# AberHu/TF-NAS

Measured on AMD Instinct MI355X. Metric: supernet search images/sec (w-step + alpha-step), higher is better.
Workload: dtype fp32

## Files before the change

include/tfnas_hip.h:

```cpp
#ifndef TFNAS_HIP_H
#define TFNAS_HIP_H

#include <stddef.h>
#include <stdint.h>

#ifdef __cplusplus
extern "C" {
#endif

#define TFNAS_ABI_VERSION 4
#define TFNAS_MAX_GROUPS 8
#define TFNAS_MAX_SINK 4
#define TFNAS_MAX_CELLS 32

#define TFNAS_MODE_CELL 0
#define TFNAS_MODE_STEM 1
#define TFNAS_MODE_HEAD 2

#define TFNAS_ACT_RELU 0
#define TFNAS_ACT_SWISH 1

#define TFNAS_EINVAL (-1)
#define TFNAS_ENULL (-2)
#define TFNAS_ERANGE (-3)
// ... 1 lines not shown
typedef struct TfnasGroup {
    int32_t mc;
    int32_t k;
    int32_t se;
    int32_t mcp;
    int32_t off;
    int32_t se_off;
    int32_t pad0, pad1;
    const float *w_expand, *w_dw, *w_proj, *w_se_r, *b_se_r, *w_se_e, *b_se_e;
    float *g_expand, *g_dw, *g_proj, *g_se_r, *gb_se_r, *g_se_e, *gb_se_e;
} TfnasGroup;

typedef struct TfnasCellDesc {
    int32_t N, H, W;
    int32_t ic, oc;
    int32_t stride;
    int32_t act;
    int32_t has_res;
    int32_t G;
    int32_t need_wgrad;
    int32_t Ho, Wo;
    int32_t M;
    int32_t SE;
    float eps;
    int32_t mode;
    int32_t Hi, Wi;
    int32_t stor;
    int32_t gemm_mode;
    int32_t flags;
    TfnasGroup g[TFNAS_MAX_GROUPS];
    int (*sync_fn)(void *user, double *table, uint64_t ndoubles, void *stream);
    void *sync_user;
    int32_t sync_world;
    int32_t route;
    int32_t fwd_route;
    int32_t pad_route;
    void *wgrad_stream[3];
} TfnasCellDesc;
#define TFNAS_GEMM_EXPLICIT 0x1000
#define TFNAS_CELL_LAZY_JOIN 1
#define TFNAS_CELL_ACCUM_WGRAD 0x20
#define TFNAS_ROUTE_FX_OFF 0x1
#define TFNAS_ROUTE_FOLD_OFF 0x2
#define TFNAS_ROUTE_DWWG_OFF 0x4
#define TFNAS_ROUTE_DWWG2_OFF 0x8
#define TFNAS_ROUTE_XG_OFF 0x10
#define TFNAS_ROUTE_XG_ALL 0x20
#define TFNAS_ROUTE_DW_SHIFT 6
#define TFNAS_ROUTE_DW_MASK 0xc0
#define TFNAS_ROUTE_SE_SHIFT 8
#define TFNAS_ROUTE_SE_MASK 0x300
#define TFNAS_ROUTE_WGRAD_INLINE 0x400
#define TFNAS_ROUTE_GRAM2 0x800
#define TFNAS_ROUTE_ALL 0xfff
#define TFNAS_ROUTE_TAKEN_VALID 0x1
#define TFNAS_ROUTE_TAKEN_FX 0x2

typedef struct TfnasCellWs {
    uint64_t E;
    uint64_t D;
    uint64_t Pr;
    uint64_t fsmall;
    uint64_t off_pooled, off_gate, off_hpre;
    uint64_t stats;
    uint64_t off_stats1, off_stats2, off_stats3;
    uint64_t out;
    uint64_t dZ;
    uint64_t dEh;
    uint64_t bsmall;
    uint64_t off_dgate, off_dpooled, off_dgl, off_dhpre, off_cb1;
    uint64_t red;
    uint64_t off_red3, off_red2, off_red1, off_resdot;
    uint64_t part;
    uint64_t dx;
    uint64_t dxp;
} TfnasCellWs;

int tfnas_abi_version(void);

typedef int (*tfnas_stats_sync_fn)(void *user, double *table, uint64_t ndoubles, void *stream);
int tfnas_set_stats_sync(tfnas_stats_sync_fn fn, void *user, int world);

int tfnas_shutdown(void);

uint64_t tfnas_sizeof(int which);

int tfnas_cell_plan(TfnasCellDesc *d);

int tfnas_cell_ws(const TfnasCellDesc *d, TfnasCellWs *ws);

int tfnas_efree_supported(const TfnasCellDesc *d);
int tfnas_cell_route(const TfnasCellDesc *d);
int tfnas_fx_supported(const TfnasCellDesc *d);

int tfnas_mixedop_fwd(const TfnasCellDesc *d, const float *x, const float *wmix,
                      float *E, float *D, float *Pr, float *fsmall, double *stats, float *part,
                      float *out, void *stream);

int tfnas_mixedop_bwd(const TfnasCellDesc *d, const float *x, const float *wmix,
                      const float *E, const float *D, const float *Pr, const float *fsmall,
                      const double *stats, const float *dout,
                      float *dZ, float *dEh, float *bsmall, double *red, float *part,
                      float *dx, float *dxp, float *dwmix, void *stream);

typedef struct TfnasBnAffine {
    const float *weight[3], *bias[3];
    float *g_weight[3], *g_bias[3];
// ... 136 lines not shown
```

tf-nas_amd/csrc/gemm_core.h:

```cpp
#pragma once
#include "tfnas_dev.h"

template <int NT>
struct GT {
    static constexpr int BM = 128, BK = 16, BN = 16 * NT;
    static constexpr int LDA = BM + 16;
    static constexpr int LDB = (BN % 32 == 16) ? BN : BN + 16;
    static constexpr int A_FLOATS = BK * LDA, B_FLOATS = BK * LDB;
    static constexpr int X3_FLOATS = 1584 * NT;
    static constexpr int LDS_FLOATS = 2 * (A_FLOATS + B_FLOATS) > X3_FLOATS ? 2 * (A_FLOATS + B_FLOATS) : X3_FLOATS;
    static constexpr int B_ITEMS = BN * 4;
    static constexpr int B_ITERS = (B_ITEMS + 255) / 256;
};

template <int NT>
__device__ __forceinline__ void acc_zero(f32x4 (&acc)[2][NT]) {
#pragma unroll
    for (int i = 0; i < 2; ++i)
#pragma unroll
        for (int j = 0; j < NT; ++j) acc[i][j] = zero4();
}

struct XfId {
    __device__ __forceinline__ f32x4 operator()(f32x4 v, int, int, int, int) const { return v; }
// ... 42 lines not shown
        _Pragma("unroll") for (int i = 0; i < T::B_ITERS; ++i) {                            \
            TFNAS_B_IDX(i);                                                                 \
            if (idx < T::B_ITEMS) {                                                         \
                const f32x4 v = xb(rb[i], (c), i, b0_, b1_);                                   \
                if (BKC) {                                                                  \
                    (Bs)[(b1_ + 0) * T::LDB + b0_] = v.x;                                   \
                    (Bs)[(b1_ + 1) * T::LDB + b0_] = v.y;                                   \
                    (Bs)[(b1_ + 2) * T::LDB + b0_] = v.z;                                   \
                    (Bs)[(b1_ + 3) * T::LDB + b0_] = v.w;                                   \
                } else {                                                                    \
                    st4(&(Bs)[b0_ * T::LDB + b1_], v);                                      \
                }                                                                           \
            }                                                                               \
        }                                                                                   \
    }

    float* As0 = lds;
    float* As1 = lds + T::A_FLOATS;
    float* Bs0 = lds + 2 * T::A_FLOATS;
    float* Bs1 = Bs0 + T::B_FLOATS;
#define TFNAS_MFMAS(As, Bs)                                                                 \
    _Pragma("unroll") for (int ks = 0; ks < 4; ++ks) {                                      \
        const int k = ks * 4 + lk;                                                          \
        const float a0 = (As)[k * T::LDA + wrow + lr];                                      \
        const float a1 = (As)[k * T::LDA + wrow + 16 + lr];                                 \
        _Pragma("unroll") for (int j = 0; j < NT; ++j) {                                    \
            const float b = (Bs)[k * T::LDB + 16 * j + lr];                                 \
            acc[0][j] = __builtin_amdgcn_mfma_f32_16x16x4f32(a0, b, acc[0][j], 0, 0, 0);    \
            acc[1][j] = __builtin_amdgcn_mfma_f32_16x16x4f32(a1, b, acc[1][j], 0, 0, 0);    \
        }                                                                                   \
    }

    if (nchunks > 0) {
        TFNAS_GLOAD(0);
        TFNAS_SSTORE(0, As0, Bs0);
    }
    __syncthreads();
    for (int c = 0; c < nchunks; ++c) {
        const bool more = (c + 1 < nchunks);
        if (more) TFNAS_GLOAD(c + 1);
        if (c & 1) { TFNAS_MFMAS(As1, Bs1); } else { TFNAS_MFMAS(As0, Bs0); }
        if (more) {
            if (c & 1) { TFNAS_SSTORE(c + 1, As0, Bs0); } else { TFNAS_SSTORE(c + 1, As1, Bs1); }
        }
        __syncthreads();
    }
#undef TFNAS_MFMAS
#undef TFNAS_GLOAD
#undef TFNAS_SSTORE
#undef TFNAS_A_IDX
#undef TFNAS_B_IDX
}

struct PreNone {
    __device__ __forceinline__ void operator()(int) const {}
};
template <int NT, bool BKC, class PRE, class LA, class XA, class LB, class XB>
__device__ __forceinline__ void gemm_mainloop_adirect(PRE& pre, LA& la, XA& xa, LB& lb, XB& xb, int nchunks,
                                                      f32x4 (&acc)[2][NT], float* lds) {
    using T = GT<NT>;
    using RA = decltype(la(0, 0, 0));
    using RB = decltype(lb(0, 0, 0));
    const int tid = threadIdx.x, lane = tid & 63;
    const int lr = lane & 15, lk = lane >> 4;
    RA ra[2];
    RB rb[T::B_ITERS];
    f32x4 cur[2];

#define TFNAS_B_IDX(i)                                                      \
    const int idx = tid + 256 * (i), b0_ = BKC ? (idx >> 2) : idx / (T::BN / 4), \
              b1_ = BKC ? (idx & 3) * 4 : (idx % (T::BN / 4)) * 4
#define TFNAS_GLOAD(c)                                                                      \
    {                                                                                       \
        pre(c);                                                                             \
        _Pragma("unroll") for (int i = 0; i < 2; ++i) ra[i] = la((c), i, 4 * lk);           \
        _Pragma("unroll") for (int i = 0; i < T::B_ITERS; ++i) {                            \
            TFNAS_B_IDX(i);                                                                 \
            if (idx < T::B_ITEMS) rb[i] = lb((c), b0_, b1_);                                \
        }                                                                                   \
    }
#define TFNAS_SSTORE(c, Bs)                                                                 \
    {                                                                                       \
        _Pragma("unroll") for (int i = 0; i < 2; ++i) cur[i] = xa(ra[i], (c), i, 4 * lk);   \
        _Pragma("unroll") for (int i = 0; i < T::B_ITERS; ++i) {                            \
            TFNAS_B_IDX(i);                                                                 \
            if (idx < T::B_ITEMS) {                                                         \
                const f32x4 v = xb(rb[i], (c), b0_, b1_);                                   \
                if (BKC) {                          \
                    const int r0_ = b1_ >> 2;                                               \
                    (Bs)[(r0_ + 0) * T::LDB + b0_] = v.x;                                   \
                    (Bs)[(r0_ + 4) * T::LDB + b0_] = v.y;                                   \
                    (Bs)[(r0_ + 8) * T::LDB + b0_] = v.z;                                   \
                    (Bs)[(r0_ + 12) * T::LDB + b0_] = v.w;                                  \
                } else {                                                                    \
                    st4(&(Bs)[((b0_ & 3) * 4 + (b0_ >> 2)) * T::LDB + b1_], v);             \
                }                                                                           \
            }                                                                               \
        }                                                                                   \
    }

    float* Bs0 = lds;
    float* Bs1 = lds + T::B_FLOATS;
    if (nchunks > 0) {
        TFNAS_GLOAD(0);
        TFNAS_SSTORE(0, Bs0);
    }
// ... 124 lines not shown
```

tf-nas_amd/csrc/gemm_kernels.hip:

```cpp
#include <stdlib.h>
#include <string.h>
#include "gemm_core.h"
#include "gemm_x3.h"
#include "kernels.h"
#include "prof.h"

__device__ __forceinline__ f32x4 stem_patch4(const float* __restrict__ img, const TfnasCellDesc& d, int p, int t0) {
    const int HW = d.H * d.W, n = p / HW, r = p - n * HW, ho = r / d.W, wo = r - ho * d.W;
    f32x4 v = zero4();
#pragma unroll
    for (int j = 0; j < 4; ++j) {
        const int t = t0 + j;
        if (t < 27) {
            const int ci = t / 9, rem = t - 9 * ci, ky = rem / 3, kx = rem - 3 * ky;
            const int hi = 2 * ho + ky - 1, wi = 2 * wo + kx - 1;
            if (hi >= 0 && hi < d.Hi && wi >= 0 && wi < d.Wi) v[j] = img[((size_t)(n * 3 + ci) * d.Hi + hi) * d.Wi + wi];
        }
    }
    return v;
}

constexpr int kLbBig = 3, kLbSmall = 4;
constexpr int kLbX3Big = 2, kLbX3Small = 3;
constexpr int gemm_lb(int nt, int mm) { return mm == 0 ? (nt >= 5 ? kLbBig : kLbSmall) : (nt >= 5 ? kLbX3Big : kLbX3Small); }
// ... 385 lines not shown
            const int pw0 = rt * 128 + w * 32;
            const int imgA = min(pw0, Po - 1) / HW, bnd = (imgA + 1) * HW;
            float sum[2][FOLD_Q][NC];
#pragma unroll
            for (int a = 0; a < 2; ++a)
#pragma unroll
                for (int q = 0; q < FOLD_Q; ++q)
#pragma unroll
                    for (int c = 0; c < NC; ++c) sum[a][q][c] = 0.f;
            const float* Dcol = D + off + n0;
            emit_tile_rows<NT>(acc, lds,
                               [&](int lrow, int lc, f32x4 v) {
                                   const int p = rt * 128 + lrow;
                                   if (p < Po && n0 + lc < mcp) st4_nt(dZ + ((size_t)p * M + off + n0 + lc), v);
                               },
                               [&](int i, const float* st) {
                                   if (d.act == TFNAS_ACT_RELU)
                                       fold_slab<NT, TFNAS_ACT_RELU>(st, LDC, Dcol, M, pw0 + 16 * i, Po, bnd, c2f, cokf, has_se, sum);
                                   else
                                       fold_slab<NT, TFNAS_ACT_SWISH>(st, LDC, Dcol, M, pw0 + 16 * i, Po, bnd, c2f, cokf, has_se, sum);
                               });
            static_assert(4 * 2 * FOLD_Q * T::BN + 4 <= T::LDS_FLOATS, "fold staging does not fit the GEMM LDS buffer");
            float* comb = lds;
            int* meta = reinterpret_cast<int*>(lds + 4 * 2 * FOLD_Q * T::BN);
#pragma unroll
            for (int a = 0; a < 2; ++a)
#pragma unroll
                for (int q = 0; q < FOLD_Q; ++q)
#pragma unroll
                    for (int c = 0; c < NC; ++c)
                        if (lane + 64 * c < T::BN) comb[((w * 2 + a) * FOLD_Q + q) * T::BN + lane + 64 * c] = sum[a][q][c];
            if (lane == 0) meta[w] = imgA;
            __syncthreads();
            const int img0 = min(rt * 128, Po - 1) / HW, imgL = min(rt * 128 + 127, Po - 1) / HW;
            const int nq = has_se ? FOLD_Q : 2;
            for (int o = tid; o < FOLD_SLOTS * FOLD_Q * T::BN; o += 256) {
                const int sl = o / (FOLD_Q * T::BN), q = (o / T::BN) % FOLD_Q, col = o % T::BN;
                if (img0 + sl > imgL || q >= nq || n0 + col >= mcp) continue;
                float t = 0.f;
#pragma unroll
                for (int ww = 0; ww < 4; ++ww)
#pragma unroll
                    for (int a = 0; a < 2; ++a)
                        if (meta[ww] + a - img0 == sl) t += comb[((ww * 2 + a) * FOLD_Q + q) * T::BN + col];
                rec[(((size_t)rt * FOLD_SLOTS + sl) * FOLD_Q + q) * M + off + n0 + col] = t;
            }
            __syncthreads();
        }
    }
}

constexpr int wgrad_lb(int nt) { return nt >= 5 ? 2 : (nt >= 3 ? 3 : 4); }

template <int NT, int ACT>
__global__ __launch_bounds__(256, wgrad_lb(NT)) void k_project_wgrad(TfnasCellDesc d, const float* __restrict__ dout,
                                                       const float* __restrict__ Pr, const float* __restrict__ D,
                                                       const float* __restrict__ gate,
                                                       const double* __restrict__ stats2,
                                                       const double* __restrict__ stats3,
                                                       const double* __restrict__ red3,
                                                       const float* __restrict__ wmix, int rows_per_split,
                                                       int ntiles_o, float* __restrict__ part, size_t out_size) {
    using T = GT<NT>;
    extern __shared__ __attribute__((aligned(16))) float lds[];
    const int g = blockIdx.z / ntiles_o, n0 = (blockIdx.z % ntiles_o) * T::BN;
    const int mc = d.g[g].mc, mcp = d.g[g].mcp, off = d.g[g].off;
    const bool has_se = d.g[g].se > 0;
    const float* gbase = has_se ? gate : D;
    const size_t se01 = has_se ? 1 : 0;
    size_t poff = 0;
    for (int gg = 0; gg < g; ++gg) poff += (size_t)d.g[gg].mc * d.oc;
    float* __restrict__ gw = part + (size_t)blockIdx.x * out_size + poff;
    const int m0 = blockIdx.y * 128;
    if (m0 >= mcp) return;
    const int HW = d.Ho * d.Wo, Po = d.N * HW, oc = d.oc, M = d.M;
    const int ocp = (oc + 15) & ~15;
    const int r0 = blockIdx.x * rows_per_split, r1 = min(Po, r0 + rows_per_split);
    const int nchunks = (r1 - r0 + 15) >> 4;
    const int tid = threadIdx.x, lane = tid & 63, lr = lane & 15, lq = lane >> 4, wrow = (tid >> 6) * 32;

    const Bn3Tab tab = bn3_tab_fill(lds + T::LDS_FLOATS, ocp, d, g, stats3, red3, wmix);
    const int mch = m0 + (tid & 31) * 4;
    const bool chok = mch < mcp;
    const size_t acol = (size_t)off + min(mch, mcp - 4);
    float2 c2[4];
#pragma unroll
    for (int j = 0; j < 4; ++j)
        c2[j] = (mch + j < mc) ? bn_consts(stats2 + 2 * (size_t)(off + mch + j), 1.0 / (double)Po, d.eps)
                               : make_float2(0.f, 0.f);
    __syncthreads();
    constexpr int BQ = T::BN / 4;
    int bcol[T::B_ITERS];
    bool bok[T::B_ITERS];
    f32x4 k_mean[T::B_ITERS], k_a3[T::B_ITERS], k_ab[T::B_ITERS], k_s[T::B_ITERS];
#pragma unroll
    for (int i = 0; i < T::B_ITERS; ++i) {
        const int idx = tid + 256 * i, o = n0 + (idx % BQ) * 4;
        bok[i] = idx < T::B_ITEMS && o < oc;
        bcol[i] = min(o, oc - 4);
#pragma unroll
        for (int j = 0; j < 4; ++j) {
            const int oo = bcol[i] + j;
            k_mean[i][j] = tab.mean[oo];
            k_a3[i][j] = tab.a3[oo];
            k_ab[i][j] = tab.a3[oo] * tab.b3[oo];
            k_s[i][j] = tab.rstd[oo] * tab.c3[oo] * tab.a3[oo];
        }
    }
    const float inv_hw = 1.f / (float)HW;
    const bool small_p = Po < (1 << 24);
    auto image_of = [&](int p) -> int {
        if (!small_p) return p / HW;
        int q = (int)((float)p * inv_hw);
        const int r = p - q * HW;
        q += (r >= HW) ? 1 : 0;
        q -= (r < 0) ? 1 : 0;
        return q;
    };

    f32x4 acc[2][NT];
    acc_zero<NT>(acc);
    auto la = [&](int c, int i, int kl, int m) -> Raw2 {
        const int p = min(r0 + c * 16 + kl, r1 - 1);
        Raw2 r;
        r.a = ld4(D + ((size_t)p * M + acol));
        r.b = ld4(gbase + ((size_t)image_of(p) * M + acol) * se01);
        return r;
    };
    auto xa = [&](Raw2 r, int c, int i, int kl, int m) -> f32x4 {
        f32x4 v = r.a;
#pragma unroll
        for (int j = 0; j < 4; ++j) v[j] = act_f<ACT>((v[j] - c2[j].x) * c2[j].y);
        if (has_se) v *= r.b;
        return (chok && r0 + c * 16 + kl < r1) ? v : zero4();
    };
    auto lb = [&](int c, int i, int kl, int n) -> Raw2 {
        const int p = min(r0 + c * 16 + kl, r1 - 1);
        Raw2 r;
        r.a = ld4(dout + (size_t)p * oc + bcol[i]);
        r.b = ld4(Pr + ((size_t)g * Po + p) * oc + bcol[i]);
        return r;
    };
    auto xb = [&](Raw2 r, int c, int i, int kl, int n) -> f32x4 {
        const f32x4 v = (k_a3[i] * r.a - k_ab[i]) - (r.b - k_mean[i]) * k_s[i];
        return (bok[i] && r0 + c * 16 + kl < r1) ? v : zero4();
    };
    gemm_mainloop2<NT, false, false, false>(la, xa, lb, xb, nchunks, acc, lds);
    const bool vec = (mc & 3) == 0;
#pragma unroll
    for (int i = 0; i < 2; ++i) {
        const int ch0 = m0 + wrow + 16 * i + 4 * lq;
#pragma unroll
        for (int j = 0; j < NT; ++j) {
            const int o = n0 + 16 * j + lr;
            if (o >= oc) continue;
            float* dst = gw + (size_t)o * mc + ch0;
            if (vec && ch0 + 3 < mc) {
                st4(dst, acc[i][j]);
            } else {
#pragma unroll
                for (int r = 0; r < 4; ++r)
                    if (ch0 + r < mc) dst[r] = acc[i][j][r];
            }
        }
    }
}

__device__ __forceinline__ f32x4 bn1_de(const f32x4* cb, f32x4 deh, f32x4 e) {
    f32x4 r;
#pragma unroll
    for (int j = 0; j < 4; ++j) {
        const f32x4 t = cb[j];
        const float eh = (e[j] - t.x) * t.y;
        r[j] = t.y * (deh[j] - t.z - eh * t.w);
    }
    return r;
}

__device__ __forceinline__ f32x4 sink_add(f32x4 v, float w, f32x4 g) {
    float px = w * g.x, py = w * g.y, pz = w * g.z, pw = w * g.w;
    asm volatile("" : "+v"(px), "+v"(py), "+v"(pz), "+v"(pw));
    f32x4 r;
    r.x = v.x + px; r.y = v.y + py; r.z = v.z + pz; r.w = v.w + pw;
    return r;
}

template <int NT, int MM>
__global__ __launch_bounds__(256, gemm_lb(NT, MM)) void k_expand_dgrad(TfnasCellDesc d, const float* __restrict__ dEh,
                                                      const float* __restrict__ x, const float* __restrict__ cb1,
                                                      const float* __restrict__ gram, const float* __restrict__ dout,
                                                      const float* __restrict__ wmix, float* __restrict__ dx,
                                                      float* __restrict__ dxp, int nsplit,
                                                      const float* __restrict__ add_src,
                                                      const float* __restrict__ add_scale, int xonly_slot = -1) {
    using T = GT<NT>;
    __shared__ __attribute__((aligned(16))) float lds[T::LDS_FLOATS];
    const int n0 = blockIdx.y * T::BN;
    const int P = d.N * d.H * d.W, ic = d.ic, M = d.M;
    const int nrt = (P + 127) >> 7;
    const int tid = threadIdx.x, lr = tid & 15, wrow = (tid >> 6) * 32;
    const int zs = (int)blockIdx.z;
    int mchunks = 0;
    for (int g = 0; g < d.G; ++g) mchunks += (d.g[g].mcp + 15) >> 4;
    const int nchunks_all = mchunks + ((ic + 15) >> 4);
    const bool xonly = xonly_slot >= 0;
    const int per = xonly ? nchunks_all - mchunks : (nchunks_all + nsplit - 1) / nsplit;
    const int cbeg = xonly ? mchunks : zs * per;
    const int nchunks = max(0, min(nchunks_all, cbeg + per) - cbeg);
    float* __restrict__ dst = xonly ? dxp + (size_t)xonly_slot * P * ic : (nsplit > 1 ? dxp + (size_t)blockIdx.z * P * ic : dx);
    const bool plain = nsplit == 1 && !xonly;
    const bool add_res = d.has_res && plain;
    const bool add_sink = add_src != nullptr && plain;
    const float sink_w = add_src ? add_scale[0] : 0.f;
    float sumw = 1.f;
    if (wmix) {
        sumw = 0.f;
// ... 550 lines not shown
}

GemmPlan gemm_plan_project_dgrad(const TfnasCellDesc& d, bool fold) {
    GemmPlan p{};
    p.var = fold ? GEMM_FOLD : GEMM_PLAIN;
    p.nt = pick_nt_groups(d);
    p.mm = gemm_arith(d, true);
    p.tiles = group_tiles(d, 16 * p.nt);
    p.grid = dim3(row_blocks(d.N * d.Ho * d.Wo, p.tiles, 1u << 30, gemm_slots(p.nt, p.mm)), p.tiles);
    p.shm = (kGtLdsFloats[p.nt] + 4 * ((d.oc + 15) & ~15)) * sizeof(float);
    return p;
}

int launch_project_dgrad(const TfnasCellDesc& d, const float* dout, const float* Pr, const double* stats3,
                         const double* red3, const float* wmix, float* dZ, hipStream_t s, const float* D,
                         const double* stats2, float* rec) {
    ProfScope _prof(TK_PROJECT_DGRAD, s);
    if (rec && (!D || !stats2)) return TFNAS_ENULL;
    const GemmPlan p = gemm_plan_project_dgrad(d, rec != nullptr);
    DISPATCH_MM(p.mm, DISPATCH_NT_GROUPS(p.nt, {
        if (p.var == GEMM_FOLD)
            hipLaunchKernelGGL((k_project_dgrad<NT, MM, true>), p.grid, dim3(256), p.shm, s, d, dout, Pr, stats3, red3, wmix, dZ,
                               D, stats2, rec);
        else
            hipLaunchKernelGGL((k_project_dgrad<NT, MM>), p.grid, dim3(256), p.shm, s, d, dout, Pr, stats3, red3, wmix, dZ);
    }))
    return (int)hipGetLastError();
}

static void plan_row_splits(GemmPlan& p, int rows, int mtiles, int ztiles, size_t scratch) {
    const int target = 256 * wgrad_lb(p.nt), min_rows = 128, out_tiles = mtiles * ztiles;
    int splits = target / (out_tiles > 0 ? out_tiles : 1);
    const size_t cap = scratch / (p.out > 0 ? p.out : 1);
    if ((size_t)splits > cap) splits = (int)cap;
    if (splits < 1) splits = 1;
    int rps = cdiv(rows, splits);
    if (rps < min_rows) rps = min_rows;
    p.rps = ((rps + 15) / 16) * 16;
    p.splits = cdiv(rows, p.rps);
    p.grid = dim3(p.splits, mtiles, ztiles);
}
static int reduce_group_wgrads(const TfnasCellDesc& d, const GemmPlan& p, const float* part, int n, float* TfnasGroup::*dst,
                               hipStream_t s) {
    size_t poff = 0;
    for (int g = 0; g < d.G; ++g) {
        const int cols = d.g[g].mc * n;
        int rc = launch_reduce_rows(part + poff, p.splits, cols, p.out, nullptr, d.g[g].*dst, s, wgrad_accum(d));
        if (rc) return rc;
        poff += cols;
    }
    return (int)hipGetLastError();
}

GemmPlan gemm_plan_project_wgrad(const TfnasCellDesc& d) {
    GemmPlan p = plan_cols(d.oc);
    p.out = mid_floats(d, d.oc);
    plan_row_splits(p, d.N * d.Ho * d.Wo, cdiv(max_mcp(d), 128), p.tiles * d.G, TFNAS_PART_FLOATS);
    p.shm = (kGtLdsFloats[p.nt] + 5 * ((d.oc + 15) & ~15)) * sizeof(float);
    return p;
}

int launch_project_wgrad(const TfnasCellDesc& d, const float* dout, const float* Pr, const float* D,
                         const float* gate, const double* stats2, const double* stats3, const double* red3,
                         const float* wmix, float* part, hipStream_t s) {
    ProfScope _prof(TK_PROJECT_WGRAD, s);
    const GemmPlan p = gemm_plan_project_wgrad(d);
    DISPATCH_NT(p.nt, DISPATCH_ACT(d.act, {
        hipLaunchKernelGGL((k_project_wgrad<NT, ACT>), p.grid, dim3(256), p.shm, s, d, dout, Pr, D, gate, stats2,
                           stats3, red3, wmix, p.rps, p.tiles, part, p.out);
    }))
    _prof.stop();
    return reduce_group_wgrads(d, p, part, d.oc, &TfnasGroup::g_proj, s);
}

size_t expand_gram_floats(const TfnasCellDesc& d) { return (size_t)(d.ic + 4) * d.ic; }
static int mid_chunks(const TfnasCellDesc& d) { return group_tiles(d, 16); }

GemmPlan gemm_plan_expand_gram(const TfnasCellDesc& d, size_t scratch_floats) {
    GemmPlan p{};
    if (!(d.route & TFNAS_ROUTE_GRAM2) && mid_floats(d, 1) <= GRAM1_MAX_K) {
        p.var = GEMM_GRAM1;
        p.grid = dim3(cdiv(d.ic, 32), cdiv(d.ic + 1, 16));
        return p;
    }
    p = plan_cols(d.ic);
    const size_t gsz = expand_gram_floats(d);
    const int mchunks = mid_chunks(d), mtiles = cdiv(d.ic + 1, 128);
    int splits = cdiv(512, mtiles * p.tiles);
    if (splits > mchunks / 4) splits = mchunks / 4;
    if ((size_t)splits > scratch_floats / gsz) splits = (int)(scratch_floats / gsz);
    if (splits < 1) splits = 1;
    p.rps = cdiv(mchunks, splits);
    p.splits = cdiv(mchunks, p.rps);
    p.grid = dim3(p.splits, mtiles, p.tiles);
    return p;
}

int launch_expand_gram(const TfnasCellDesc& d, const float* cb1, float* scratch, size_t scratch_floats, float* gram,
                       hipStream_t s) {
    ProfScope _prof(TK_SMALL, s);
    const GemmPlan p = gemm_plan_expand_gram(d, scratch_floats);
    if (p.var == GEMM_GRAM1) {
        for (int g = 0; g < d.G; ++g)
            if (d.g[g].mc < 1) return TFNAS_EINVAL;
        if (d.mode == TFNAS_MODE_HEAD) hipLaunchKernelGGL(k_gram1<16>, p.grid, dim3(1024), 0, s, d, cb1, gram);
        else hipLaunchKernelGGL(k_gram1<4>, p.grid, dim3(256), 0, s, d, cb1, gram);
        return (int)hipGetLastError();
    }
    const size_t gsz = expand_gram_floats(d);
    if (scratch_floats < gsz) return TFNAS_ERANGE;
    DISPATCH_NT(p.nt, { hipLaunchKernelGGL(k_expand_gram<NT>, p.grid, dim3(256), 0, s, d, cb1, p.rps, p.splits, scratch); })
    _prof.stop();
    return launch_reduce_rows(scratch, p.splits, (int)gsz, gsz, nullptr, gram, s);
}

GemmPlan gemm_plan_expand_dgrad(const TfnasCellDesc& d, bool split, int nsl) {
    GemmPlan p = plan_cols(d.ic);
    p.mm = gemm_arith(d, true);
    const int P = d.N * d.H * d.W, out_tiles = cdiv(P, 128) * p.tiles;
    p.splits = 1;
    if (split && nsl < 0 && out_tiles < 512) {
        const int mchunks = mid_chunks(d);
        int ns = cdiv(1024, out_tiles);
        if (ns > 16) ns = 16;
        if (ns > mchunks / 4) ns = mchunks / 4;
        if (d.need_wgrad && d.G == 1 && ns > TFNAS_WSPLIT_DGRAD) ns = TFNAS_WSPLIT_DGRAD;
// ... 66 lines not shown
```

tf-nas_amd/csrc/kernels.h:

```cpp
#pragma once
#include <stdlib.h>
#include <hip/hip_runtime.h>
#include "tfnas_hip.h"

struct StatsSync {
    tfnas_stats_sync_fn fn;
    void* user;
    int world;
};
extern StatsSync g_stats_sync;
static inline StatsSync sync_of(const TfnasCellDesc& d) {
    if (d.sync_fn) return StatsSync{d.sync_fn, d.sync_user, d.sync_world > 0 ? d.sync_world : 1};
    return g_stats_sync;
}
static inline bool stats_sync_on(const TfnasCellDesc& d) { return sync_of(d).fn != nullptr; }
static inline int stats_sync(const TfnasCellDesc& d, double* table, size_t ndoubles, hipStream_t s) {
    const StatsSync y = sync_of(d);
    return y.fn ? y.fn(y.user, table, (uint64_t)ndoubles, (void*)s) : 0;
}
static inline uint64_t stats_world(const TfnasCellDesc& d) {
    const StatsSync y = sync_of(d);
    return (y.fn && y.world > 1) ? (uint64_t)y.world : 1;
}

static inline int route_dw(const TfnasCellDesc& d) { return (d.route & TFNAS_ROUTE_DW_MASK) >> TFNAS_ROUTE_DW_SHIFT; }
static inline int route_se(const TfnasCellDesc& d) { return (d.route & TFNAS_ROUTE_SE_MASK) >> TFNAS_ROUTE_SE_SHIFT; }
static inline bool route_side(const TfnasCellDesc& d) { return !(d.route & TFNAS_ROUTE_WGRAD_INLINE); }
static inline int wgrad_accum(const TfnasCellDesc& d) { return (d.flags & TFNAS_CELL_ACCUM_WGRAD) ? 1 : 0; }
#define ACT_DISPATCH(act, ...)                                                          \
    if ((act) == TFNAS_ACT_RELU) { constexpr int ACT = TFNAS_ACT_RELU; __VA_ARGS__; }   \
    else { constexpr int ACT = TFNAS_ACT_SWISH; __VA_ARGS__; }

int gemm_mode();
int set_gemm_mode(int m);
int gemm_mode_of(const TfnasCellDesc& d);
enum GemmVariant { GEMM_PLAIN, GEMM_STEM, GEMM_XG, GEMM_FOLD, GEMM_GRAM1 };
struct GemmPlan {
    GemmVariant var;
    int mm;
    int nt, tiles;
    int splits;
    int rps;
    int parts;
    dim3 grid, grid2;
    size_t shm;
    size_t out, out_main;
};
GemmPlan gemm_plan_expand_fwd(const TfnasCellDesc& d);
GemmPlan gemm_plan_project_fwd(const TfnasCellDesc& d);
GemmPlan gemm_plan_project_dgrad(const TfnasCellDesc& d, bool fold);
GemmPlan gemm_plan_project_wgrad(const TfnasCellDesc& d);
GemmPlan gemm_plan_expand_gram(const TfnasCellDesc& d, size_t scratch_floats);
GemmPlan gemm_plan_expand_dgrad(const TfnasCellDesc& d, bool split, int nsl = -1);
GemmPlan gemm_plan_expand_wgrad(const TfnasCellDesc& d);
int launch_expand_fwd(const TfnasCellDesc& d, const float* x, float* E, double* stats1, float* part,
                      hipStream_t s);
int launch_project_fwd(const TfnasCellDesc& d, const float* D, const float* gate, const double* stats2,
                       float* Pr, double* stats3, float* part, hipStream_t s);
int launch_project_dgrad(const TfnasCellDesc& d, const float* dout, const float* Pr, const double* stats3,
                         const double* red3, const float* wmix, float* dZ, hipStream_t s, const float* D = nullptr,
                         const double* stats2 = nullptr, float* rec = nullptr);
constexpr int FOLD_SLOTS = 4, FOLD_Q = 5;
static inline bool project_fold_ok(const TfnasCellDesc& d, size_t scratch_floats) {
    const int HW = d.Ho * d.Wo;
    const size_t nrt = ((size_t)d.N * HW + 127) / 128;
    return HW >= 43 && nrt * FOLD_SLOTS * FOLD_Q * (size_t)d.M <= scratch_floats;
}
int launch_project_wgrad(const TfnasCellDesc& d, const float* dout, const float* Pr, const float* D,
                         const float* gate, const double* stats2, const double* stats3, const double* red3,
                         const float* wmix, float* part, hipStream_t s);
size_t expand_gram_floats(const TfnasCellDesc& d);
int launch_expand_gram(const TfnasCellDesc& d, const float* cb1, float* scratch, size_t scratch_floats, float* gram,
                       hipStream_t s);
int launch_expand_dgrad(const TfnasCellDesc& d, const float* dEh, const float* x, const float* cb1, const float* gram,
                        const float* dout, const float* wmix, float* dx, float* dxp, hipStream_t s,
                        const float* add_src = nullptr, const float* add_scale = nullptr, int nsl = -1);
int launch_expand_wgrad(const TfnasCellDesc& d, const float* dEh, const float* E, const float* cb1,
                        const float* x, float* part, hipStream_t s);

struct DwDirect {
    int chunks;
    int ncg;
    int nseg;
    int per;
    int steps;
    int nwg;
};
struct DwSlide {
    int TH, TW;
    int CC, CCP, cq_shift;
    int RB, L1;
    int chunks, gx;
};
// ... 107 lines not shown
```

tf-nas_amd/tfnas_amd/_lib.py:

```python
import ctypes as C
import os

import torch

_HERE = os.path.dirname(os.path.abspath(__file__))
LIB_PATH = os.environ.get('TFNAS_LIB') or os.path.join(_HERE, 'libtfnas_hip.so')

MAX_GROUPS, MAX_SINK, MAX_CELLS = 8, 4, 32
ACT = {'relu': 0, 'swish': 1}
MODE_CELL, MODE_STEM, MODE_HEAD = 0, 1, 2

_W_FIELDS = ('w_expand', 'w_dw', 'w_proj', 'w_se_r', 'b_se_r', 'w_se_e', 'b_se_e')
_G_FIELDS = ('g_expand', 'g_dw', 'g_proj', 'g_se_r', 'gb_se_r', 'g_se_e', 'gb_se_e')


GEMM_EXPLICIT, GEMM_EVERYWHERE, CELL_LAZY_JOIN = 0x1000, 0x100, 1
CELL_ACCUM_WGRAD = 0x20
ROUTE_FX_OFF, ROUTE_FOLD_OFF, ROUTE_DWWG_OFF, ROUTE_DWWG2_OFF, ROUTE_XG_OFF, ROUTE_XG_ALL = 0x1, 0x2, 0x4, 0x8, 0x10, 0x20
ROUTE_DW = {'auto': 0, 'direct': 1 << 6, 'lds': 2 << 6, 'tiled': 3 << 6}
ROUTE_SE = {'wave': 0, 'fused': 1 << 8, 'gemm': 2 << 8}
ROUTE_WGRAD_INLINE, ROUTE_GRAM2 = 0x400, 0x800
ROUTE_TAKEN_VALID, ROUTE_TAKEN_FX = 1, 2
GEMM_MODES = {'f32': 0, 'bf16': 1, 'x2': 3, 'x3': 6}


class TfnasGroup(C.Structure):
    _fields_ = ([(n, C.c_int32) for n in ('mc', 'k', 'se', 'mcp', 'off', 'se_off', 'pad0', 'pad1')]
                + [(n, C.c_void_p) for n in _W_FIELDS] + [(n, C.c_void_p) for n in _G_FIELDS])


class TfnasCellDesc(C.Structure):
    _fields_ = ([(n, C.c_int32) for n in ('N', 'H', 'W', 'ic', 'oc', 'stride', 'act', 'has_res', 'G', 'need_wgrad',
                                          'Ho', 'Wo', 'M', 'SE')]
                + [('eps', C.c_float), ('mode', C.c_int32), ('Hi', C.c_int32), ('Wi', C.c_int32),
                   ('stor', C.c_int32), ('gemm_mode', C.c_int32), ('flags', C.c_int32), ('g', TfnasGroup * MAX_GROUPS),
                   ('sync_fn', C.c_void_p), ('sync_user', C.c_void_p), ('sync_world', C.c_int32), ('route', C.c_int32),
                   ('fwd_route', C.c_int32), ('pad_route', C.c_int32), ('wgrad_stream', C.c_void_p * 3)])


class TfnasCellWs(C.Structure):
    _fields_ = [(n, C.c_uint64) for n in (
        'E', 'D', 'Pr', 'fsmall', 'off_pooled', 'off_gate', 'off_hpre', 'stats', 'off_stats1', 'off_stats2',
        'off_stats3', 'out', 'dZ', 'dEh', 'bsmall', 'off_dgate', 'off_dpooled', 'off_dgl', 'off_dhpre', 'off_cb1',
        'red', 'off_red3', 'off_red2', 'off_red1', 'off_resdot', 'part', 'dx', 'dxp')]


MAX_STAGES = 8


class TfnasStage(C.Structure):
    _fields_ = ([(n, C.c_int32) for n in ('ncell', 'start_res', 'first_cell', 'nres')]
                + [('betas', C.c_void_p), ('dbetas', C.c_void_p)])


class TfnasPathDesc(C.Structure):
    _fields_ = ([(n, C.c_int32) for n in ('ncell', 'nstage', 'soft', 'need_dx0', 'efree_mask_lo', 'reserved0')]
                + [('stage', TfnasStage * MAX_STAGES), ('cell', TfnasCellDesc * MAX_CELLS)])


class TfnasPathWs(C.Structure):
    _fields_ = ([(n, C.c_uint64) for n in ('saved', 'scratch', 'total', 'out_count')]
                + [(n, C.c_int32) for n in ('out_h', 'out_w', 'out_c', 'pad')])


class TfnasBnAffine(C.Structure):
    _fields_ = ([(n, C.c_void_p * 3) for n in ('weight', 'bias', 'g_weight', 'g_bias', 'running_mean', 'running_var')]
                + [('momentum', C.c_float), ('eval', C.c_int32)])


_P = C.c_void_p
_PP = C.POINTER(C.c_void_p)
_PROTOS = {
    'tfnas_abi_version': (C.c_int, []),
    'tfnas_shutdown': (C.c_int, []),
# ... 111 lines not shown
```

tf-nas_amd/tfnas_amd/functions.py:

```python
import ctypes as C
import os

import torch

from . import _lib
from ._lib import TfnasCellDesc, TfnasCellWs, ptr, ptr_array, check

BN_EPS = 1e-5
_EFREE_ENV = os.environ.get('TFNAS_EFREE', '1')
EFREE = _EFREE_ENV != '0'
EFREE_STRIDE1 = _EFREE_ENV == 'all'


def route_from_env(env=None):
    env = os.environ if env is None else env
    r = 0
    for var, bit in (('TFNAS_FX', _lib.ROUTE_FX_OFF), ('TFNAS_FOLD', _lib.ROUTE_FOLD_OFF), ('TFNAS_DWWG', _lib.ROUTE_DWWG_OFF),
                     ('TFNAS_DWWG2', _lib.ROUTE_DWWG2_OFF), ('TFNAS_WGRAD_STREAM', _lib.ROUTE_WGRAD_INLINE)):
        if env.get(var, '1')[:1] == '0':
            r |= bit
    xg = env.get('TFNAS_XG', 'auto')
    r |= _lib.ROUTE_XG_OFF if xg[:1] == '0' else (_lib.ROUTE_XG_ALL if xg == 'all' else 0)
    r |= _lib.ROUTE_DW.get(env.get('TFNAS_DW', 'auto'), 0) | _lib.ROUTE_SE.get(env.get('TFNAS_SE', 'wave'), 0)
    if env.get('TFNAS_GRAM', '1') == '2':
        r |= _lib.ROUTE_GRAM2
    return r


def route_bits(fx=True, fold=True, dwwg=True, dwwg2=True, xg='auto', dw='auto', se='wave', wgrad_stream=True, gram=1):
    return route_from_env({'TFNAS_FX': '1' if fx else '0', 'TFNAS_FOLD': '1' if fold else '0', 'TFNAS_DWWG': '1' if dwwg else '0',
                           'TFNAS_DWWG2': '1' if dwwg2 else '0', 'TFNAS_XG': xg, 'TFNAS_DW': dw, 'TFNAS_SE': se,
                           'TFNAS_WGRAD_STREAM': '1' if wgrad_stream else '0', 'TFNAS_GRAM': str(gram)})


ENV_ROUTE = route_from_env()


def _stream(dev):
    return C.c_void_p(torch.cuda.current_stream(dev).cuda_stream)


class _Null:
    def __enter__(self):
        return None

    def __exit__(self, *a):
        return False


_NULL = _Null()


def _on(dev):
    return _NULL if torch.cuda.current_device() == dev.index else torch.cuda.device(dev)


def _same_device(dev, tensors, what):
    for t in tensors:
        if t is not None and t.device != dev:
            raise RuntimeError('tfnas_amd: %s lives on %s but the input is on %s -- all operands of a launch must share '
                               'one device (one process per GPU; nn.DataParallel replicas must own their parameters)'
                               % (what, t.device, dev))


def _nhwc(x):
    v = x.permute(0, 2, 3, 1)
    return v if v.is_contiguous() else v.contiguous()


def _require_cuda(t, what):
    if not t.is_cuda:
        raise RuntimeError('tfnas_amd: %s must live on the GPU -- the MixedOP hot path has no CPU implementation '
                           '(the CPU restatement is oracle/tfnas_oracle.py, test infrastructure only)' % what)
    if t.dtype != torch.float32:
        raise RuntimeError('tfnas_amd: %s must be float32' % what)


def _no_plan():
    return None


class HipModes:

    def __init__(self, gemm=None, everywhere=False, lazy_join=False, direct_grads=False, sync=None, route=None):
        self.gemm, self.everywhere, self.lazy_join, self.direct_grads, self.sync = gemm, everywhere, lazy_join, direct_grads, sync
# ... 544 lines not shown
```

Baseline: 3893.

## Use narrow-M tiles with split-K reduction for small-channel projection weight gradients

Adds a GEMM mainloop variant for the projection weight-gradient kernel that uses 32- or 64-row M tiles when the mid-channel count is small. Each wave covers a different K slice, and the partial accumulators are reduced through LDS before the stores. The goal is to stop wasting most of a 128-row tile on padding for narrow layers, and to do more K work per chunk. The variant applies only to single-group cells with up to 48 output columns. It adds an LDS reduction pass and more template instantiations, and the old behaviour can be forced back with a route bit.

```diff
diff --git a/include/tfnas_hip.h b/include/tfnas_hip.h
--- a/include/tfnas_hip.h
+++ b/include/tfnas_hip.h
@@ -77,7 +77,8 @@
 #define TFNAS_ROUTE_SE_MASK 0x300
 #define TFNAS_ROUTE_WGRAD_INLINE 0x400
 #define TFNAS_ROUTE_GRAM2 0x800
-#define TFNAS_ROUTE_ALL 0xfff
+#define TFNAS_ROUTE_PWG_WIDE 0x2000
+#define TFNAS_ROUTE_ALL 0x2fff
 #define TFNAS_ROUTE_TAKEN_VALID 0x1
 #define TFNAS_ROUTE_TAKEN_FX 0x2
 
diff --git a/tf-nas_amd/csrc/gemm_core.h b/tf-nas_amd/csrc/gemm_core.h
--- a/tf-nas_amd/csrc/gemm_core.h
+++ b/tf-nas_amd/csrc/gemm_core.h
@@ -118,6 +118,93 @@
 #undef TFNAS_B_IDX
 }
 
+constexpr int gtk_lds_floats(int nt, int mt) {
+    const int ab = 2 * (16 * 144 + (2048 / mt) * 16 * nt), red = 4 * 2 * nt * 256;
+    return ab > red ? ab : red;
+}
+template <int NT, int MT>
+struct GTK {
+    static constexpr int KQ = 128 / MT, KS = 16 * KQ, BN = 16 * NT;
+    static constexpr int LDA = GT<NT>::LDA, LDB = BN;
+    static constexpr bool SWZ = BN % 32 == 0;
+    static constexpr int A_FLOATS = 16 * LDA, B_FLOATS = KS * LDB;
+    static constexpr int LDS_FLOATS = gtk_lds_floats(NT, MT);
+    static constexpr int B_ITEMS = KS * BN / 4;
+    static constexpr int B_ITERS = (B_ITEMS + 255) / 256;
+};
+
+template <int NT, int MT, class LA, class XA, class LB, class XB>
+__device__ __forceinline__ void gemm_mainloop_kq(LA& la, XA& xa, LB& lb, XB& xb, int nchunks, f32x4 (&acc)[2][NT], float* lds) {
+    using T = GTK<NT, MT>;
+    static_assert((MT == 32 || MT == 64) && NT <= 3 && T::LDA == 144, "narrow tiles: 32 or 64 rows, at most 48 columns");
+    static_assert(2 * (T::A_FLOATS + T::B_FLOATS) <= T::LDS_FLOATS && (T::BN % 32 == 16 || T::BN == 32), "B tile layout");
+    using RA = decltype(la(0, 0, 0, 0));
+    using RB = decltype(lb(0, 0, 0, 0));
+    const int tid = threadIdx.x, lane = tid & 63, wrow = (tid >> 6) * 32;
+    const int lr = lane & 15, lk = lane >> 4;
+    const int acol = (tid & 31) * 4, akk = (acol / MT) * 16 + (tid >> 5), am = acol % MT;
+    const int bq = (wrow / MT) * 16;
+    constexpr int BQ = T::BN / 4;
+    RA ra[2];
+    RB rb[T::B_ITERS];
+
+#define TFNAS_GLOAD(c)                                                                      \
+    {                                                                                       \
+        _Pragma("unroll") for (int i = 0; i < 2; ++i) ra[i] = la((c), i, akk + 8 * i, am);  \
+        _Pragma("unroll") for (int i = 0; i < T::B_ITERS; ++i) {                            \
+            const int idx = tid + 256 * i;                                                  \
+            rb[i] = lb((c), i, idx / BQ, (idx % BQ) * 4);                                   \
+        }                                                                                   \
+    }
+#define TFNAS_SSTORE(c, As, Bs)                                                             \
+    {                                                                                       \
+        _Pragma("unroll") for (int i = 0; i < 2; ++i) {                                     \
+            const f32x4 v = xa(ra[i], (c), i, akk + 8 * i, am);                             \
+            st4(&(As)[((tid >> 5) + 8 * i) * T::LDA + acol], v);                            \
+        }                                                                                   \
+        _Pragma("unroll") for (int i = 0; i < T::B_ITERS; ++i) {                            \
+            const int idx = tid + 256 * i, kk = idx / BQ, n = (idx % BQ) * 4;               \
+            if (idx < T::B_ITEMS) {                                                         \
+                const f32x4 v = xb(rb[i], (c), i, kk, n);                                   \
+                st4(&(Bs)[kk * T::LDB + (T::SWZ ? n ^ ((kk & 1) << 4) : n)], v);            \
+            }                                                                               \
+        }                                                                                   \
+    }
+#define TFNAS_MFMAS(As, Bs)                                                                 \
+    _Pragma("unroll") for (int ks = 0; ks < 4; ++ks) {                                      \
+        const int k = ks * 4 + lk;                                                          \
+        const float a0 = (As)[k * T::LDA + wrow + lr];                                      \
+        const float a1 = (As)[k * T::LDA + wrow + 16 + lr];                                 \
+        _Pragma("unroll") for (int j = 0; j < NT; ++j) {                                    \
+            const int col = 16 * j + lr;                                                    \
+            const float b = (Bs)[(bq + k) * T::LDB + (T::SWZ ? col ^ ((k & 1) << 4) : col)]; \
+            acc[0][j] = __builtin_amdgcn_mfma_f32_16x16x4f32(a0, b, acc[0][j], 0, 0, 0);    \
+            acc[1][j] = __builtin_amdgcn_mfma_f32_16x16x4f32(a1, b, acc[1][j], 0, 0, 0);    \
+        }                                                                                   \
+    }
+    float* As0 = lds;
+    float* As1 = lds + T::A_FLOATS;
+    float* Bs0 = lds + 2 * T::A_FLOATS;
+    float* Bs1 = Bs0 + T::B_FLOATS;
+    if (nchunks > 0) {
+        TFNAS_GLOAD(0);
+        TFNAS_SSTORE(0, As0, Bs0);
+    }
+    __syncthreads();
+    for (int c = 0; c < nchunks; ++c) {
+        const bool more = (c + 1 < nchunks);
+        if (more) TFNAS_GLOAD(c + 1);
+        if (c & 1) { TFNAS_MFMAS(As1, Bs1); } else { TFNAS_MFMAS(As0, Bs0); }
+        if (more) {
+            if (c & 1) { TFNAS_SSTORE(c + 1, As0, Bs0); } else { TFNAS_SSTORE(c + 1, As1, Bs1); }
+        }
+        __syncthreads();
+    }
+#undef TFNAS_MFMAS
+#undef TFNAS_GLOAD
+#undef TFNAS_SSTORE
+}
+
 struct PreNone {
     __device__ __forceinline__ void operator()(int) const {}
 };
diff --git a/tf-nas_amd/csrc/gemm_kernels.hip b/tf-nas_amd/csrc/gemm_kernels.hip
--- a/tf-nas_amd/csrc/gemm_kernels.hip
+++ b/tf-nas_amd/csrc/gemm_kernels.hip
@@ -461,7 +461,7 @@
 
 constexpr int wgrad_lb(int nt) { return nt >= 5 ? 2 : (nt >= 3 ? 3 : 4); }
 
-template <int NT, int ACT>
+template <int NT, int ACT, int MT = 128>
 __global__ __launch_bounds__(256, wgrad_lb(NT)) void k_project_wgrad(TfnasCellDesc d, const float* __restrict__ dout,
                                                        const float* __restrict__ Pr, const float* __restrict__ D,
                                                        const float* __restrict__ gate,
@@ -471,6 +471,9 @@
                                                        const float* __restrict__ wmix, int rows_per_split,
                                                        int ntiles_o, float* __restrict__ part, size_t out_size) {
     using T = GT<NT>;
+    constexpr int KS = 16 * (128 / MT);
+    constexpr int LDSF = MT == 128 ? T::LDS_FLOATS : gtk_lds_floats(NT, MT);
+    constexpr int B_ITEMS = KS * T::BN / 4, NB = (B_ITEMS + 255) / 256;
     extern __shared__ __attribute__((aligned(16))) float lds[];
     const int g = blockIdx.z / ntiles_o, n0 = (blockIdx.z % ntiles_o) * T::BN;
     const int mc = d.g[g].mc, mcp = d.g[g].mcp, off = d.g[g].off;
@@ -480,16 +483,16 @@
     size_t poff = 0;
     for (int gg = 0; gg < g; ++gg) poff += (size_t)d.g[gg].mc * d.oc;
     float* __restrict__ gw = part + (size_t)blockIdx.x * out_size + poff;
-    const int m0 = blockIdx.y * 128;
+    const int m0 = blockIdx.y * MT;
     if (m0 >= mcp) return;
     const int HW = d.Ho * d.Wo, Po = d.N * HW, oc = d.oc, M = d.M;
     const int ocp = (oc + 15) & ~15;
     const int r0 = blockIdx.x * rows_per_split, r1 = min(Po, r0 + rows_per_split);
-    const int nchunks = (r1 - r0 + 15) >> 4;
+    const int nchunks = (r1 - r0 + KS - 1) / KS;
     const int tid = threadIdx.x, lane = tid & 63, lr = lane & 15, lq = lane >> 4, wrow = (tid >> 6) * 32;
 
-    const Bn3Tab tab = bn3_tab_fill(lds + T::LDS_FLOATS, ocp, d, g, stats3, red3, wmix);
-    const int mch = m0 + (tid & 31) * 4;
+    const Bn3Tab tab = bn3_tab_fill(lds + LDSF, ocp, d, g, stats3, red3, wmix);
+    const int mch = m0 + ((tid & 31) * 4) % MT;
     const bool chok = mch < mcp;
     const size_t acol = (size_t)off + min(mch, mcp - 4);
     float2 c2[4];
@@ -499,13 +502,13 @@
                                : make_float2(0.f, 0.f);
     __syncthreads();
     constexpr int BQ = T::BN / 4;
-    int bcol[T::B_ITERS];
-    bool bok[T::B_ITERS];
-    f32x4 k_mean[T::B_ITERS], k_a3[T::B_ITERS], k_ab[T::B_ITERS], k_s[T::B_ITERS];
-#pragma unroll
-    for (int i = 0; i < T::B_ITERS; ++i) {
+    int bcol[NB];
+    bool bok[NB];
+    f32x4 k_mean[NB], k_a3[NB], k_ab[NB], k_s[NB];
+#pragma unroll
+    for (int i = 0; i < NB; ++i) {
         const int idx = tid + 256 * i, o = n0 + (idx % BQ) * 4;
-        bok[i] = idx < T::B_ITEMS && o < oc;
+        bok[i] = idx < B_ITEMS && o < oc;
         bcol[i] = min(o, oc - 4);
 #pragma unroll
         for (int j = 0; j < 4; ++j) {
@@ -530,7 +533,7 @@
     f32x4 acc[2][NT];
     acc_zero<NT>(acc);
     auto la = [&](int c, int i, int kl, int m) -> Raw2 {
-        const int p = min(r0 + c * 16 + kl, r1 - 1);
+        const int p = min(r0 + c * KS + kl, r1 - 1);
         Raw2 r;
         r.a = ld4(D + ((size_t)p * M + acol));
         r.b = ld4(gbase + ((size_t)image_of(p) * M + acol) * se01);
@@ -541,10 +544,10 @@
 #pragma unroll
         for (int j = 0; j < 4; ++j) v[j] = act_f<ACT>((v[j] - c2[j].x) * c2[j].y);
         if (has_se) v *= r.b;
-        return (chok && r0 + c * 16 + kl < r1) ? v : zero4();
+        return (chok && r0 + c * KS + kl < r1) ? v : zero4();
     };
     auto lb = [&](int c, int i, int kl, int n) -> Raw2 {
-        const int p = min(r0 + c * 16 + kl, r1 - 1);
+        const int p = min(r0 + c * KS + kl, r1 - 1);
         Raw2 r;
         r.a = ld4(dout + (size_t)p * oc + bcol[i]);
         r.b = ld4(Pr + ((size_t)g * Po + p) * oc + bcol[i]);
@@ -552,25 +555,42 @@
     };
     auto xb = [&](Raw2 r, int c, int i, int kl, int n) -> f32x4 {
         const f32x4 v = (k_a3[i] * r.a - k_ab[i]) - (r.b - k_mean[i]) * k_s[i];
-        return (bok[i] && r0 + c * 16 + kl < r1) ? v : zero4();
+        return (bok[i] && r0 + c * KS + kl < r1) ? v : zero4();
     };
-    gemm_mainloop2<NT, false, false, false>(la, xa, lb, xb, nchunks, acc, lds);
+    if constexpr (MT == 128) gemm_mainloop2<NT, false, false, false>(la, xa, lb, xb, nchunks, acc, lds);
+    else gemm_mainloop_kq<NT, MT>(la, xa, lb, xb, nchunks, acc, lds);
     const bool vec = (mc & 3) == 0;
-#pragma unroll
-    for (int i = 0; i < 2; ++i) {
-        const int ch0 = m0 + wrow + 16 * i + 4 * lq;
-#pragma unroll
-        for (int j = 0; j < NT; ++j) {
-            const int o = n0 + 16 * j + lr;
-            if (o >= oc) continue;
-            float* dst = gw + (size_t)o * mc + ch0;
-            if (vec && ch0 + 3 < mc) {
-                st4(dst, acc[i][j]);
-            } else {
-#pragma unroll
-                for (int r = 0; r < 4; ++r)
-                    if (ch0 + r < mc) dst[r] = acc[i][j][r];
-            }
+    auto put = [&](int ch0, int o, f32x4 v) {
+        if (o >= oc) return;
+        float* dst = gw + (size_t)o * mc + ch0;
+        if (vec && ch0 + 3 < mc) {
+            st4(dst, v);
+        } else {
+#pragma unroll
+            for (int r = 0; r < 4; ++r)
+                if (ch0 + r < mc) dst[r] = v[r];
+        }
+    };
+    if constexpr (MT == 128) {
+#pragma unroll
+        for (int i = 0; i < 2; ++i)
+#pragma unroll
+            for (int j = 0; j < NT; ++j) put(m0 + wrow + 16 * i + 4 * lq, n0 + 16 * j + lr, acc[i][j]);
+    } else {
+        constexpr int BANDS = MT / 32, KQ = 4 / BANDS;
+        static_assert(4 * 2 * NT * 256 <= LDSF, "the waves' accumulators do not fit the GEMM LDS buffer");
+        f32x4* red = reinterpret_cast<f32x4*>(lds);
+        const int w = tid >> 6, band = w % BANDS;
+#pragma unroll
+        for (int i = 0; i < 2; ++i)
+#pragma unroll
+            for (int j = 0; j < NT; ++j) red[((w * 2 + i) * NT + j) * 64 + lane] = acc[i][j];
+        __syncthreads();
+        for (int it = w / BANDS; it < 2 * NT; it += KQ) {
+            f32x4 v = red[(band * 2 * NT + it) * 64 + lane];
+#pragma unroll
+            for (int q = 1; q < KQ; ++q) v += red[((band + q * BANDS) * 2 * NT + it) * 64 + lane];
+            put(m0 + 32 * band + 16 * (it / NT) + 4 * lq, n0 + 16 * (it % NT) + lr, v);
         }
     }
 }
@@ -1227,26 +1247,41 @@
     return (int)hipGetLastError();
 }
 
+static constexpr int PWG_NARROW_MAX = 64, PWG_CLASS96_MT = 32;
 GemmPlan gemm_plan_project_wgrad(const TfnasCellDesc& d) {
     GemmPlan p = plan_cols(d.oc);
     p.out = mid_floats(d, d.oc);
-    plan_row_splits(p, d.N * d.Ho * d.Wo, cdiv(max_mcp(d), 128), p.tiles * d.G, TFNAS_PART_FLOATS);
-    p.shm = (kGtLdsFloats[p.nt] + 5 * ((d.oc + 15) & ~15)) * sizeof(float);
+    const int mcp = max_mcp(d);
+    p.mt = 128;
+    if (d.G == 1 && !(d.route & TFNAS_ROUTE_PWG_WIDE) && p.nt <= 3 && mcp <= PWG_NARROW_MAX)
+        p.mt = (mcp <= 32 && p.nt < 3) ? 32 : (mcp <= 64 ? 64 : PWG_CLASS96_MT);
+    plan_row_splits(p, d.N * d.Ho * d.Wo, cdiv(mcp, p.mt), p.tiles * d.G, TFNAS_PART_FLOATS);
+    p.shm = ((p.mt == 128 ? kGtLdsFloats[p.nt] : gtk_lds_floats(p.nt, p.mt)) + 5 * ((d.oc + 15) & ~15)) * sizeof(float);
     return p;
 }
 
+#define PWG_LAUNCH(MT_)                                                                                                  \
+    hipLaunchKernelGGL((k_project_wgrad<NT, ACT, MT_>), p.grid, dim3(256), p.shm, s, d, dout, Pr, D, gate, stats2, stats3, \
+                       red3, wmix, p.rps, p.tiles, part, p.out)
 int launch_project_wgrad(const TfnasCellDesc& d, const float* dout, const float* Pr, const float* D,
                          const float* gate, const double* stats2, const double* stats3, const double* red3,
                          const float* wmix, float* part, hipStream_t s) {
     ProfScope _prof(TK_PROJECT_WGRAD, s);
     const GemmPlan p = gemm_plan_project_wgrad(d);
-    DISPATCH_NT(p.nt, DISPATCH_ACT(d.act, {
-        hipLaunchKernelGGL((k_project_wgrad<NT, ACT>), p.grid, dim3(256), p.shm, s, d, dout, Pr, D, gate, stats2,
-                           stats3, red3, wmix, p.rps, p.tiles, part, p.out);
-    }))
+    if (p.mt == 128) {
+        DISPATCH_NT(p.nt, DISPATCH_ACT(d.act, { PWG_LAUNCH(128); }))
+    } else {
+        switch (p.nt) {
+            NT_CASE(1, DISPATCH_ACT(d.act, { if (p.mt == 32) PWG_LAUNCH(32); else PWG_LAUNCH(64); }))
+            NT_CASE(2, DISPATCH_ACT(d.act, { if (p.mt == 32) PWG_LAUNCH(32); else PWG_LAUNCH(64); }))
+            NT_CASE(3, DISPATCH_ACT(d.act, { PWG_LAUNCH(64); }))
+            default: return TFNAS_EINVAL;
+        }
+    }
     _prof.stop();
     return reduce_group_wgrads(d, p, part, d.oc, &TfnasGroup::g_proj, s);
 }
+#undef PWG_LAUNCH
 
 size_t expand_gram_floats(const TfnasCellDesc& d) { return (size_t)(d.ic + 4) * d.ic; }
 static int mid_chunks(const TfnasCellDesc& d) { return group_tiles(d, 16); }
diff --git a/tf-nas_amd/csrc/kernels.h b/tf-nas_amd/csrc/kernels.h
--- a/tf-nas_amd/csrc/kernels.h
+++ b/tf-nas_amd/csrc/kernels.h
@@ -39,6 +39,7 @@
     GemmVariant var;
     int mm;
     int nt, tiles;
+    int mt;
     int splits;
     int rps;
     int parts;
diff --git a/tf-nas_amd/tfnas_amd/_lib.py b/tf-nas_amd/tfnas_amd/_lib.py
--- a/tf-nas_amd/tfnas_amd/_lib.py
+++ b/tf-nas_amd/tfnas_amd/_lib.py
@@ -20,6 +20,7 @@
 ROUTE_DW = {'auto': 0, 'direct': 1 << 6, 'lds': 2 << 6, 'tiled': 3 << 6}
 ROUTE_SE = {'wave': 0, 'fused': 1 << 8, 'gemm': 2 << 8}
 ROUTE_WGRAD_INLINE, ROUTE_GRAM2 = 0x400, 0x800
+ROUTE_PWG_WIDE = 0x2000
 ROUTE_TAKEN_VALID, ROUTE_TAKEN_FX = 1, 2
 GEMM_MODES = {'f32': 0, 'bf16': 1, 'x2': 3, 'x3': 6}
 
diff --git a/tf-nas_amd/tfnas_amd/functions.py b/tf-nas_amd/tfnas_amd/functions.py
--- a/tf-nas_amd/tfnas_amd/functions.py
+++ b/tf-nas_amd/tfnas_amd/functions.py
@@ -24,13 +24,15 @@
     r |= _lib.ROUTE_DW.get(env.get('TFNAS_DW', 'auto'), 0) | _lib.ROUTE_SE.get(env.get('TFNAS_SE', 'wave'), 0)
     if env.get('TFNAS_GRAM', '1') == '2':
         r |= _lib.ROUTE_GRAM2
+    if env.get('TFNAS_PWG', 'auto') == 'wide':
+        r |= _lib.ROUTE_PWG_WIDE
     return r
 
 
-def route_bits(fx=True, fold=True, dwwg=True, dwwg2=True, xg='auto', dw='auto', se='wave', wgrad_stream=True, gram=1):
+def route_bits(fx=True, fold=True, dwwg=True, dwwg2=True, xg='auto', dw='auto', se='wave', wgrad_stream=True, gram=1, pwg='auto'):
     return route_from_env({'TFNAS_FX': '1' if fx else '0', 'TFNAS_FOLD': '1' if fold else '0', 'TFNAS_DWWG': '1' if dwwg else '0',
                            'TFNAS_DWWG2': '1' if dwwg2 else '0', 'TFNAS_XG': xg, 'TFNAS_DW': dw, 'TFNAS_SE': se,
-                           'TFNAS_WGRAD_STREAM': '1' if wgrad_stream else '0', 'TFNAS_GRAM': str(gram)})
+                           'TFNAS_WGRAD_STREAM': '1' if wgrad_stream else '0', 'TFNAS_GRAM': str(gram), 'TFNAS_PWG': pwg})
 
 
 ENV_ROUTE = route_from_env()
```

Measured after the change: 3883. About the same (-0.3%).
